# YukeWang96/GNNAdvisor_OSDI21

Measured on AMD Instinct MI355X. Metric: aggregated edges/sec, GCN sum-aggregation SpMM (SAG) hidden=64, higher is better.
Workload: dtype f32; 1 GPU; reddit-like power-law graph, random node order; num_nodes=232965, nnz=114623790, dim=64, partSize=128, num_parts=1008217, parallelism=single GPU, call=GNNA.SAG (pybind module, reference signature, fresh output), decider=auto/mi355x, column_phases=16, build_id=0.6.1+9562461010c46275

## Files before the change

gnnadvisor_osdi21_amd/csrc/gnna_agg.hip:

```cpp
#include <hip/hip_runtime.h>

#include <algorithm>
#include <cmath>
#include <cstdint>
#include <cstdio>

#include "gnna.h"
#include "gnna_device.h"
#include "gnna_internal.h"

namespace gnna {
namespace {


__global__ void __launch_bounds__(kBlock)
prologue_kernel(float *__restrict__ Y, size_t n_floats, int D, int ldy, const int32_t *__restrict__ p2n,
                const int32_t *__restrict__ pp, int64_t P, int32_t *flag, int32_t seq, int validate, int zero_fill,
                const int32_t *__restrict__ chk_ids, int64_t chk_n, const unsigned long long *__restrict__ chk_sum,
                int32_t *stale_flag, uint32_t *__restrict__ clear_words, int n_clear)
{
    if (blockIdx.x == 0 && (int)threadIdx.x < n_clear) clear_words[threadIdx.x] = 0u;
    const unsigned fill_blocks = chk_ids ? gridDim.x - 1 : gridDim.x;
    if (blockIdx.x >= fill_blocks) {
        if (threadIdx.x < kWave) {
// ... 90 lines not shown
        const bool valid = g < P;
        int64_t lo = 0, cnt = 0;
        if (valid) {
            const int64_t r = p2n[g];
            const int64_t nxt = g + 1 < P ? (int64_t)p2n[g + 1] : N;
            const int a = pp[g], b = pp[g + 1];
            if (b < a || (g + 1 < P && nxt < r)) bad = true;
            const bool continues = g > 0 && (g % G) == 0 && p2n[g - 1] == r;
            const bool self = b <= a || continues;
            lo = self ? r : r + 1;
            int64_t hi = (self && nxt < r + 1) ? r + 1 : nxt;
            lo = lo < 0 ? 0 : lo;
            hi = hi > N ? N : hi;
            cnt = hi > lo ? hi - lo : 0;
        }
        unsigned long long m = __ballot(cnt > 0);
        while (m) {
            const int l = __builtin_ctzll(m);
            m &= m - 1;
            const int64_t lo_s = ((int64_t)__builtin_amdgcn_readlane((int)(lo >> 32), l) << 32) |
                                 (uint32_t)__builtin_amdgcn_readlane((int)lo, l);
            const int64_t cnt_s = ((int64_t)__builtin_amdgcn_readlane((int)(cnt >> 32), l) << 32) |
                                  (uint32_t)__builtin_amdgcn_readlane((int)cnt, l);
            clear_rows(lo_s, cnt_s);
        }
    }
    if (validate && bad) *flag = seq;
}

__global__ void __launch_bounds__(kBlock)
post_prologue_kernel(float *__restrict__ Y, size_t n_floats, int D, int ldy, const int32_t *flag, int32_t seq,
                     const unsigned long long *gaps)
{
    const size_t tid = (size_t)blockIdx.x * blockDim.x + threadIdx.x;
    const size_t nthreads = (size_t)gridDim.x * blockDim.x;
    auto at = [&](float *base, size_t i) -> float * {
        if (ldy == D) return base + i;
        const size_t r = i / (unsigned)D;
        return base + r * (size_t)ldy + (i - r * (unsigned)D);
    };
    if (*flag == seq) {
        for (size_t i = tid; i < n_floats; i += nthreads) *at(Y, i) = 0.f;
        return;
    }
    if (!gaps) return;
    const unsigned long long n = gaps[0] < (unsigned long long)kGapEntries ? gaps[0] : (unsigned long long)kGapEntries;
    for (unsigned long long k = 0; k < n; k++) {
        float *base = Y + (size_t)gaps[2 + 2 * k] * (size_t)ldy;
        const size_t cnt = (size_t)gaps[3 + 2 * k] * (size_t)D;
        for (size_t i = tid; i < cnt; i += nthreads) *at(base, i) = 0.f;
    }
}

__global__ void __launch_bounds__(kBlock)
scale_rows_kernel(const float *__restrict__ X, int64_t ld_in, const float *__restrict__ deg, float *__restrict__ Xs,
                  int64_t rows, int D, int ld_out)
{
    const size_t tid = (size_t)blockIdx.x * blockDim.x + threadIdx.x;
    const size_t nthreads = (size_t)gridDim.x * blockDim.x;
    typedef float f32x4 __attribute__((ext_vector_type(4)));
    const bool aligned = ((reinterpret_cast<uintptr_t>(X) | reinterpret_cast<uintptr_t>(Xs)) & 15) == 0;
    if (ld_out == D && ld_in == D && (D & 3) == 0 && aligned) {
        const size_t n4 = ((size_t)rows * (size_t)D) >> 2;
        const int d4 = D >> 2;
        for (size_t i = tid; i < n4; i += nthreads) {
            const f32x4 v = __builtin_nontemporal_load(reinterpret_cast<const f32x4 *>(X) + i);
            reinterpret_cast<f32x4 *>(Xs)[i] = deg ? v * deg[i / d4] : v;
        }
    } else if ((D & 3) == 0 && (ld_out & 3) == 0 && (ld_in & 3) == 0 && aligned) {
        const size_t n4 = ((size_t)rows * (size_t)D) >> 2;
        const unsigned d4 = (unsigned)D >> 2;
        const size_t ldo4 = (size_t)ld_out >> 2, ldi4 = (size_t)ld_in >> 2;
        for (size_t i = tid; i < n4; i += nthreads) {
            const size_t r = i / d4, c4 = i - r * d4;
            const f32x4 v = __builtin_nontemporal_load(reinterpret_cast<const f32x4 *>(X) + r * ldi4 + c4);
            reinterpret_cast<f32x4 *>(Xs)[r * ldo4 + c4] = deg ? v * deg[r] : v;
        }
    } else {
        const size_t total = (size_t)rows * (size_t)D;
        for (size_t i = tid; i < total; i += nthreads) {
            const size_t r = i / (unsigned)D, cc = i - r * (unsigned)D;
            const float v = __builtin_nontemporal_load(X + r * (size_t)ld_in + cc);
            Xs[r * (size_t)ld_out + cc] = deg ? v * deg[r] : v;
        }
    }
}


static size_t gather_footprint_bytes(int64_t num_in_rows, int ldx, int dim)
{
    return (size_t)num_in_rows * (size_t)std::min(ldx, (std::max(dim, 4) * 4 + 127) / 128 * 32) * sizeof(float);
}

thread_local int t_last_phases = 1;
thread_local int t_last_launches = 1;

double avg_lines_per_row(int64_t row_bytes, int64_t stride_bytes)
{
    int64_t lines = 0;
    for (int k = 0; k < 32; k++) {
        const int64_t o = (k * stride_bytes) % 128;
        lines += (o + row_bytes + 127) / 128;
    }
    return (double)lines / 32.0;
}

int choose_row_stride(int dim)
{
    if (dim < 2 || dim > 256) return dim;
    auto cost = [&](int stride) {
        return avg_lines_per_row((int64_t)dim * 4, (int64_t)stride * 4) * ((stride & 3) ? 1.07 : 1.0);
    };
    const double plain = cost(dim);
    int best = dim;
    double best_cost = plain * 0.93;
    const int cand[3] = {(dim + 3) / 4 * 4, (dim + 15) / 16 * 16, (dim + 31) / 32 * 32};
    for (int c : cand) {
        if (c == dim || c > 2 * dim) continue;
        const double cc = cost(c) * (1.0 + 0.02 * (double)(c - dim) / (double)dim);
        if (cc < best_cost) { best = c; best_cost = cc; }
    }
    return best;
}

int pick_row_stride(const gnna_tuning &t, int dim, bool hot_rows, int64_t num_in_rows, bool whole_call)
{
    int ldx = dim;
    if (t.pad_rows == 1 || (t.pad_rows == 0 && hot_rows)) ldx = choose_row_stride(dim);
    if (t.pad_rows == 0 && hot_rows && dim > 16 && dim <= 64 && whole_call) {
        const int gapped = 2 * ((dim * 4 + 127) / 128) * 32;
        if ((size_t)num_in_rows * (size_t)gapped * sizeof(float) <= ((size_t)160 << 20)) ldx = gapped;
    }
    if (t.pad_rows > 2 && t.pad_rows >= dim) ldx = t.pad_rows;
    return ldx;
}

}
// ... 230 lines not shown
            int64_t blocks = (num_parts + kBlock - 1) / kBlock;
            blocks = std::max<int64_t>(1, std::min<int64_t>(blocks, (int64_t)ds->num_cus * 8));
            unsigned long long *gaps = ds->gap_lists + (size_t)call_block_of(ds, stream, seq) * kGapWords;
            (void)hipMemsetAsync(gaps, 0, sizeof(unsigned long long), stream);
            const int64_t big_rows = std::max<int64_t>(64, ((int64_t)1 << 20) / std::max(1, dim * 4));
            hipLaunchKernelGGL(sparse_prologue_kernel, dim3((unsigned)blocks), dim3(kBlock), 0, stream, out, num_nodes, dim, ldy,
                               part2Node, part_pointers, num_parts, sparse_G, flag, seq, validate, gaps, big_rows);
            hipLaunchKernelGGL(post_prologue_kernel, dim3((unsigned)(ds->num_cus * 8)), dim3(kBlock), 0, stream, out,
                               n_floats, dim, ldy, flag, seq, gaps);
        } else {
            size_t work = std::max(n_floats / 4, (size_t)num_parts);
            int64_t blocks = (int64_t)((work + kBlock - 1) / kBlock);
            blocks = std::max<int64_t>(1, std::min<int64_t>(blocks, (int64_t)ds->num_cus * 8));
            hipLaunchKernelGGL(prologue_kernel, dim3((unsigned)blocks + (chk_sum ? 1u : 0u)), dim3(kBlock), 0, stream, out, n_floats,
                               dim, ldy, part2Node, part_pointers, num_parts, flag, seq, validate, zero_fill,
                               chk_sum ? column_index : nullptr, chk_n, chk_sum, stale_flag, clear_words, n_clear);
        }
        hipError_t e = hipGetLastError();
        if (e != hipSuccess) return fail(GNNA_ERR_HIP, "prologue launch: %s", hipGetErrorString(e));
        profile_record(prof_call, 1, stream);
        return GNNA_OK;
    };
    if (num_parts == 0) {
        rc = run_prologue(0);
        if (rc != GNNA_OK || !relu || !accumulate_into_out) return rc;
        StreamLaunch e0;
        e0.mode = mode; e0.Y = out; e0.p2n = part2Node; e0.P = 0; e0.D = dim; e0.ldy = ldy; e0.relu = true; e0.num_out_rows = num_nodes;
        e0.flag = flag; e0.seq = seq; e0.cnt = nullptr; e0.B = 1; e0.plain_ok = false; e0.G = 1;
        return launch_stream_epilogue_only(e0, stream);
    }

    const int64_t window_rows = (num_in_rows + num_windows - 1) / num_windows;

    const int64_t est_edges = num_parts * (int64_t)(tune.avg_degree > 0 ? std::min(partSize, tune.avg_degree) : partSize / 2 + 1);
    const bool hot_rows = est_edges >= 32 * num_in_rows && (size_t)num_in_rows * (size_t)dim * sizeof(float) <= ((size_t)1 << 30);
    const bool prescale = mode == MODE_GCN && (tune.gcn_prescale == 1 || (tune.gcn_prescale == 0 && hot_rows));
    const int want = dim < 4 ? 4 : pick_row_stride(tune, dim, hot_rows, num_in_rows, !windowed);
    bool direct = !prescale && dim >= 4;
    if (direct && want != dim && ld_in != want) {
        const bool aligned16 = (reinterpret_cast<uintptr_t>(input) & 15) == 0 && (ld_in & 3) == 0;
        const int gapped = 2 * ((dim * 4 + 127) / 128) * 32;
        if (want == gapped && dim > 16 && dim <= 64)
            direct = (ld_in % gapped) == 0 && (reinterpret_cast<uintptr_t>(input) % ((size_t)gapped * 4)) == 0;
        else
            direct = aligned16 && avg_lines_per_row((int64_t)dim * 4, ld_in * 4) <= avg_lines_per_row((int64_t)dim * 4, (int64_t)want * 4) + 1e-9;
    }
    const int ldx = direct ? (int)ld_in : want;
    const float *X = input;
    const float *row_scale = nullptr;
    float eps = epsilon;
    const size_t x_bytes = (size_t)num_in_rows * (size_t)ldx * sizeof(float);
    const size_t foot_bytes = gather_footprint_bytes(num_in_rows, ldx, dim);
    const bool wide = x_bytes > 0xffffffffull;
    if (!direct) {
        void *xs = nullptr;
        rc = get_workspace(ds, stream, 1, x_bytes, &xs);
        if (rc != GNNA_OK) return rc;
        const int64_t r0 = std::min<int64_t>((int64_t)win_begin * window_rows, num_in_rows);
        const int64_t r1 = std::min<int64_t>((int64_t)win_end * window_rows, num_in_rows);
        const size_t s_bytes = (size_t)(r1 - r0) * (size_t)dim * sizeof(float);
        int64_t sblocks = (int64_t)((s_bytes / 16 + kBlock - 1) / kBlock);
        sblocks = std::max<int64_t>(1, std::min<int64_t>(sblocks, (int64_t)ds->num_cus * 8));
        hipLaunchKernelGGL(scale_rows_kernel, dim3((unsigned)sblocks), dim3(kBlock), 0, stream,
                           input + (size_t)r0 * (size_t)ld_in, ld_in, prescale ? degrees_in + r0 : nullptr,
                           static_cast<float *>(xs) + (size_t)r0 * ldx, r1 - r0, dim, ldx);
        hipError_t es = hipGetLastError();
        if (es != hipSuccess) return fail(GNNA_ERR_HIP, "staging launch: %s", hipGetErrorString(es));
        X = static_cast<const float *>(xs);
        if (prescale) {
            row_scale = degrees;
            eps = 1.f;
            mode = MODE_GIN;
        }
    }

    int B = 1;
    const uint8_t *cnt = nullptr;
    int S = kMaxSlices;
    int win_lo = 0, win_hi = 0;
    SlicePlan plan;
    const bool can_slice = num_parts >= 1024 && num_in_rows >= 64 && foot_bytes >= ((size_t)2 << 20);
    if (windowed) {
        rc = get_slice_plan(ds, stream, column_index, part_pointers, part2Node, num_parts, num_in_rows, true, false, &plan,
                            (uint32_t)std::max<int64_t>(1, window_rows));
        if (rc != GNNA_OK) return rc;
        if (!plan.cnt || !plan.stats.valid)
            return fail(GNNA_ERR_UNSUPPORTED, "the windowed aggregation needs its window counts, which cannot be built inside a "
                                              "stream capture: run the sequence once before capturing it");
        if (plan.stats.unsorted > 0)
            return fail(GNNA_ERR_UNSUPPORTED, "windowed aggregation: the column ids of %.0f neighbor-groups are not in increasing "
                                              "order (sort the ids of every row, as the loader's CSR has them)", plan.stats.unsorted);
        cnt = plan.cnt; S = plan.S; B = 1;
        win_lo = win_begin; win_hi = win_end == num_windows ? S : win_end;
    } else {
        if (tune.column_phases >= 2 && num_in_rows >= kMaxSlices) {
            B = std::min(tune.column_phases, kMaxSlices);
            rc = get_slice_plan(ds, stream, column_index, part_pointers, part2Node, num_parts, num_in_rows, false, false, &plan);
            if (rc != GNNA_OK) return rc;
        } else if (tune.column_phases == 0 && can_slice && foot_bytes >= ((size_t)6 << 20)) {
            rc = get_slice_plan(ds, stream, column_index, part_pointers, part2Node, num_parts, num_in_rows, true, false, &plan);
            if (rc != GNNA_OK) return rc;
            if (plan.cnt && plan.stats.valid)
                B = choose_slices(plan.stats, foot_bytes, plan.S, plan.slice_rows, num_nodes, num_in_rows == num_nodes,
                                  tune.nonlocal_ids == 1);
        }
        cnt = plan.cnt;
        if (cnt) S = plan.S;
        if (!cnt || B < 2) { B = 1; cnt = nullptr; }
    }

    const int auto_Bs = (cnt && !windowed && plan.stats.valid)
                            ? sweep_auto_phases(tune, mode, dim, foot_bytes, num_nodes, num_in_rows, plan.stats, B, ds->num_cus,
                                                tune.deterministic == 1, partSize) : 0;
    if (mode != MODE_EDGE && cnt && !windowed && dim >= 4 && (tune.sweep == 1 || auto_Bs > 0) && tune.deterministic != 1 &&
        sweep_supports(mode, dim, x_bytes)) {
        int Bs = B;
        if (auto_Bs > 0) {
            Bs = std::min(auto_Bs, S);
        } else if (tune.column_phases < 2) {
            Bs = std::max(2, std::min(std::min(std::min(16, 2 * B), std::max(2, partSize / 4)), S));
        }
        const int32_t *sw_ids = nullptr; const uint32_t *sw_off = nullptr;
        if (plan.handle && (tune.pack_ids == 1 || (tune.pack_ids == 0 && plan.pinned)) && tune.xcd_remap != 0) {
            rc = get_packed_ids(ds, stream, plan.handle, Bs, kWave, true, false, &sw_ids, &sw_off, &chk_sum, &chk_n, stale_flag, seq,
                                tune.ids_check_every);
            if (rc != GNNA_OK) return rc;
            if (sw_ids) count_event(CTR_PACKED_LAUNCHES);
        }
        uint32_t *sync = ds->sweep_sync + (size_t)call_block_of(ds, stream, seq) * kSweepSlotWords;
        static_assert(kXcds * 16 + 2 <= kBlock, "the prologue clears the sweep counters with one block");
        rc = run_prologue(0, sync, kXcds * 16 + 2);
        if (rc != GNNA_OK) return rc;
        SweepLaunch w;
        w.mode = mode; w.X = X; w.col = column_index; w.pp = part_pointers; w.p2n = part2Node; w.Y = out;
        w.cnt = cnt; w.row_scale = row_scale; w.flag = flag; w.seq = seq; w.trust = tune.trust_canonical ? 1 : 0; w.sync = sync;
        w.P = num_parts; w.D = dim; w.ldx = ldx; w.ldy = ldy; w.S = S; w.B = Bs;
        w.relu = relu; w.num_out_rows = num_nodes;
        w.U = std::max(tune.loads_in_flight, 8);
        w.rows_with_edges = plan.stats.valid ? (int64_t)std::min((double)num_nodes, plan.stats.groups) : num_nodes;
        if (tune.groups_per_chunk > 64) w.rounds = tune.groups_per_chunk / 64;
        w.slack = tune.sweep_slack; w.wgs_per_cu = tune.blocks_per_cu;
        w.dynamic = tune.xcd_remap != 0;
        w.plain_ok = !accumulate_into_out; w.eps = eps;
        w.ids_packed = sw_ids; w.item_off = sw_off; w.packed_stale = stale_flag;
        t_last_phases = Bs;
        t_last_launches = 1;
        rc = launch_sweep(ds, w, stream);
        if (rc != GNNA_OK) return rc;
        profile_record(prof_call, 2, stream);
        return GNNA_OK;
    }

    int G = std::min(64, tune.groups_per_chunk * B);
    if (mode == MODE_EDGE && cnt && !windowed && plan.handle && plan.pinned && (plan.stats.valid || tune.sweep == 1) &&
        tune.xcd_remap != 0) {
        const int Bs = sweep_phases_of_width(tune, dim, foot_bytes, x_bytes, num_nodes, num_in_rows, plan.stats, B, ds->num_cus,
                                             partSize, S);
        if (Bs >= 2) { B = Bs; G = kWave; }
    }
    t_last_phases = B;
    StreamLaunch a;
    a.mode = mode; a.X = X; a.col = column_index; a.pp = part_pointers; a.p2n = part2Node; a.Y = out;
    a.cnt = cnt; a.row_scale = row_scale; a.flag = flag; a.seq = seq;
    if (mode == MODE_EDGE) { a.deg_row = nullptr; a.deg_col = nullptr; a.edge_w = degrees_in; }
    else { a.deg_row = degrees; a.deg_col = degrees_in; }
    a.trust = tune.trust_canonical ? 1 : 0; a.P = num_parts;
    a.D = dim; a.ldx = ldx; a.ldy = ldy; a.G = G; a.U = tune.loads_in_flight; a.S = S; a.B = B;
    a.win_lo = win_lo; a.win_hi = win_hi; a.relu = relu; a.num_out_rows = num_nodes;
    t_last_launches = 1;
    a.wide = wide; a.plain_ok = (B == 1 && !accumulate_into_out && !windowed); a.xcd_remap = tune.xcd_remap != 0;
    a.eps = eps;
    if (tune.deterministic == 1 && !windowed) {
        const int G_eff = std::max(1, std::min(a.G, kWave));
        const size_t chunks = (size_t)((num_parts + G_eff - 1) / G_eff);
        const size_t part_bytes = ((chunks * 2 * (size_t)dim * sizeof(float)) + 255) & ~(size_t)255;
        const size_t stamp_bytes = chunks * 2 * sizeof(int32_t);
        void *ws = nullptr;
        rc = get_workspace(ds, stream, 2, part_bytes + stamp_bytes, &ws);
        if (rc != GNNA_OK) return rc;
        a.det = true;
        a.det_part = static_cast<float *>(ws);
        a.det_stamp = reinterpret_cast<int32_t *>(static_cast<char *>(ws) + part_bytes);
        hipError_t em = hipMemsetAsync(a.det_stamp, 0, stamp_bytes, stream);
        if (em != hipSuccess) return fail(GNNA_ERR_HIP, "deterministic schedule scratch: %s", hipGetErrorString(em));
        t_last_launches = B;
    }
    if (cnt && !windowed && plan.handle && (tune.pack_ids == 1 || (tune.pack_ids == 0 && plan.pinned))) {
        rc = get_packed_ids(ds, stream, plan.handle, B, std::max(1, std::min(a.G, kWave)), true, false, &a.ids_packed, &a.item_off,
                            &chk_sum, &chk_n, stale_flag, seq, tune.ids_check_every);
        a.packed_stale = stale_flag;
        if (rc != GNNA_OK) return rc;
        if (a.ids_packed) count_event(CTR_PACKED_LAUNCHES);
    }
    const bool sparse = !a.det && a.plain_ok && tune.zero_fill != 2 &&
                        (tune.zero_fill == 1 || n_floats * sizeof(float) >= ((size_t)32 << 20));
    rc = run_prologue(sparse ? std::max(1, std::min(a.G, kWave)) : 0);
    if (rc != GNNA_OK) return rc;
    rc = launch_stream(a, stream);
    if (rc != GNNA_OK) return rc;
    profile_record(prof_call, 2, stream);
    return GNNA_OK;
}

}
}
// ... 283 lines not shown
```

gnnadvisor_osdi21_amd/csrc/gnna_device.h:

```cpp
#ifndef GNNA_DEVICE_H_
#define GNNA_DEVICE_H_

#include <hip/hip_runtime.h>

#include <cstdint>
#include <type_traits>

namespace gnna {


constexpr int kWave = 64;
constexpr int kBlock = 256;
constexpr int kWavesPerBlock = kBlock / kWave;
constexpr int kXcds = 8;

enum { MODE_SAG = 0, MODE_GCN = 1, MODE_GIN = 2, MODE_SDDMM = 3, MODE_EDGE = 4 };

template <int VEC> struct VecOf;
template <> struct VecOf<1> { typedef float T; typedef float M; };
template <> struct VecOf<4> {
    typedef float T __attribute__((ext_vector_type(4)));
    typedef T M __attribute__((aligned(4)));
};

// ... 87 lines not shown
        float px, qy;
        {
            auto t = __builtin_amdgcn_permlane32_swap(__float_as_uint(acc[0]), __float_as_uint(acc[2]), false, false);
            px = __uint_as_float(t[0]) + __uint_as_float(t[1]);
            t = __builtin_amdgcn_permlane32_swap(__float_as_uint(acc[1]), __float_as_uint(acc[3]), false, false);
            qy = __uint_as_float(t[0]) + __uint_as_float(t[1]);
        }
        float val;
        {
            auto t = __builtin_amdgcn_permlane16_swap(__float_as_uint(px), __float_as_uint(qy), false, false);
            val = __uint_as_float(t[0]) + __uint_as_float(t[1]);
        }
        if constexpr (LPR <= 8) val += row_ror<8>(val);
        if constexpr (LPR <= 4) val += row_ror<4>(val);
        if constexpr (MODE == MODE_GIN) val *= scale;
        r[0] = val;
    } else {
#pragma unroll
        for (int k = 0; k < 4; k++) {
            float s = slot_reduce<LPR>(acc[k]);
            if constexpr (MODE == MODE_GIN) s *= scale;
            r[k] = s;
        }
    }
    return r;
}

__device__ __forceinline__ unsigned long long sample_checksum(const int32_t *__restrict__ ids, int64_t n, int lane)
{
    unsigned long long sum = 0;
    if (n > 0) {
        uint32_t v[16];
#pragma unroll
        for (int k = 0; k < 16; k++) {
            const int i = k * 64 + lane;
            v[k] = (uint32_t)ids[(int64_t)(((unsigned long long)i * (unsigned long long)n) >> 10)];
        }
#pragma unroll
        for (int k = 0; k < 16; k++) sum += (unsigned long long)v[k] * (unsigned long long)(2 * (k * 64 + lane) + 1);
    }
    for (int d = 32; d > 0; d >>= 1) sum += __shfl_xor(sum, d);
    return sum;
}

__device__ __forceinline__ unsigned long long graph_checksum(const int32_t *__restrict__ ids, int64_t n,
                                                             const int32_t *__restrict__ pp, int64_t P, int lane)
{
    const unsigned long long a = sample_checksum(ids, n, lane);
    const unsigned long long b = sample_checksum(pp, P + 1, lane);
    const unsigned long long last = (unsigned long long)(uint32_t)pp[P];
    return a ^ ((b + last) * 0x9E3779B97F4A7C15ull);
}

}

#endif
```

gnnadvisor_osdi21_amd/csrc/gnna_internal.h:

```cpp
#ifndef GNNA_INTERNAL_H_
#define GNNA_INTERNAL_H_

#include <hip/hip_runtime.h>

#include <atomic>
#include <cstddef>
#include <cstdint>
#include <map>
#include <utility>
#include <vector>

#include "gnna.h"

namespace gnna {

int fail(int code, const char *fmt, ...) __attribute__((format(printf, 2, 3)));

int host_thread_budget(int cap);

void apply_graph_hints(const void *column_index, int dim, gnna_tuning *tune);

struct Workspace {
    void *ptr = nullptr;
    size_t bytes = 0;
// ... 82 lines not shown
       CTR_COUNT = 10 };
void count_event(int which);

struct StreamLaunch {
    int mode;
    const float *X; const int32_t *col; const int32_t *pp; const int32_t *p2n; float *Y;
    const uint8_t *cnt;
    const float *row_scale;
    const float *deg_row; const float *deg_col;
    const float *A = nullptr;
    const float *edge_w = nullptr;
    const int32_t *flag; int32_t seq; int32_t trust;
    int64_t P;
    int D, ldx, G, U, S, B;
    int lda = 0;
    int ldy = 0;
    int win_lo = 0, win_hi = 0;
    bool relu = false;
    int64_t num_out_rows = 0;
    bool wide, plain_ok, xcd_remap;
    float eps;
    bool det = false;
    float *det_part = nullptr; int32_t *det_stamp = nullptr;
    const int32_t *ids_packed = nullptr; const uint32_t *item_off = nullptr;
    const int32_t *packed_stale = nullptr;
};
int launch_stream(const StreamLaunch &a, hipStream_t stream);
int launch_stream_epilogue_only(const StreamLaunch &a, hipStream_t stream);

struct SweepLaunch {
    int mode;
    const float *X; const int32_t *col; const int32_t *pp; const int32_t *p2n; float *Y;
    const uint8_t *cnt;
    const float *row_scale;
    const int32_t *flag; int32_t seq; int32_t trust;
    uint32_t *sync;
    int64_t P;
    int D, ldx, U, S, B;
    int ldy = 0;
    bool relu = false;
    int64_t num_out_rows = 0;
    int rounds = 0;
    int64_t rows_with_edges = 0;
    int slack = 0;
    int wgs_per_cu = 0;
    bool dynamic = true;
    bool plain_ok;
    float eps;
    const int32_t *ids_packed = nullptr; const uint32_t *item_off = nullptr;
    const int32_t *packed_stale = nullptr;
};
bool sweep_supports(int mode, int dim, size_t x_bytes);
int sweep_acc_rows(int dim, int wgs_per_cu);
int launch_sweep(DeviceState *ds, const SweepLaunch &a, hipStream_t stream);
int sweep_auto_phases(const gnna_tuning &t, int mode, int dim, size_t x_bytes, int64_t num_out_rows, int64_t num_in_rows,
                      const SlicePlanStats &st, int B, int num_cus, bool deterministic, int part_size);
constexpr int kSweepListCap = 1023;
constexpr int kSweepSlotWords = 8 * 16 + 2 + 2 * kSweepListCap;

struct X16Launch {
    int mode;
    int in_type, out_type;
    const void *input; int64_t ld_in, num_in_rows;
    const int32_t *column_index; const float *degrees_out; const float *degrees_in; float epsilon;
    const int32_t *part_pointers; const int32_t *part2Node;
    void *out; int64_t ld_out, num_out_rows;
    int dim; int64_t num_parts; int partSize;
    bool accumulate, relu, xcd_remap;
    int prof_call = -1;
};
int launch_x16(DeviceState *ds, hipStream_t stream, const X16Launch &c);
int reserve_x16(DeviceState *ds, hipStream_t stream, int64_t num_in_rows, int64_t num_out_rows, int dim);
int launch_zero_fill(DeviceState *ds, hipStream_t stream, float *out, int64_t rows, int dim, int64_t ld);

int64_t scan_tiles(int64_t n);
int launch_exclusive_scan(hipStream_t stream, int32_t *data, int64_t n, int32_t *partial);
int refuse_capture(const char *what, hipStream_t stream);

int profile_acquire_call(bool has_work);
void profile_record(int call, int which, hipStream_t stream);

}

#endif
```

gnnadvisor_osdi21_amd/csrc/gnna_sweep.hip:

```cpp
#include <hip/hip_runtime.h>

#include <algorithm>
#include <cmath>
#include <cstdint>

#include "gnna.h"
#include "gnna_device.h"
#include "gnna_internal.h"

namespace gnna {
namespace {

constexpr int kSweepIdSlots = 512;
constexpr int kSweepBlock = 1024;
constexpr int kSweepWaves = kSweepBlock / kWave;
constexpr int kSweepLockWords = 128;

template <int LPR, int WGS> constexpr int acc_floats()
{
    return WGS == 1 ? (LPR >= 16 ? 32768 : 28672) : (LPR >= 16 ? 15360 : 11264);
}

__device__ __forceinline__ void lds_add(float *p, float v)
{
    typedef __attribute__((address_space(3))) float lds_float;
    (void)__hip_atomic_fetch_add((lds_float *)p, v, __ATOMIC_RELAXED, __HIP_MEMORY_SCOPE_WORKGROUP);
}

struct SweepParams {
    const float *X;
    const int32_t *col;
    const int32_t *pp;
    const int32_t *p2n;
    float *Y;
    const uint8_t *cnt;
    const float *row_scale;
    const int32_t *flag;
    uint32_t *sync;
    int64_t P;
    int32_t seq;
    int32_t trust;
    int32_t D;
    int32_t ldx;
    int32_t ldy;
    int32_t relu;
    int32_t S;
    int32_t B;
    int32_t rounds;
    int32_t plain_ok;
    int32_t dynamic;
    int32_t slack;
    float eps;
    const int32_t *ids_packed;
    const uint32_t *item_off;
    const int32_t *packed_stale;
    int64_t num_chunks;
};

__device__ __forceinline__ int64_t lower_bound64(const int32_t *__restrict__ pp, int64_t P, int64_t target, int lane)
{
    int64_t lo = 0, hi = P;
    while (hi > lo) {
        const int64_t span = hi - lo;
        const int64_t idx = lo + (span * lane) / kWave;
        const bool below = (int64_t)pp[idx] < target;
        const int c = __popcll(__ballot(below));
        if (c == 0) { hi = lo; break; }
        const int64_t new_lo = lo + (span * (c - 1)) / kWave + 1;
        const int64_t new_hi = c < kWave ? lo + (span * c) / kWave : hi;
        lo = new_lo;
        hi = new_hi > new_lo ? new_hi : new_lo;
    }
    return lo;
}

__device__ __forceinline__ int64_t sweep_set_start(int64_t i, int64_t num_sets, int64_t nnz, const int32_t *__restrict__ pp,
                                                   int64_t P, bool canonical, bool align64, int lane)
{
    const int64_t target = i >= num_sets ? nnz : (nnz * i) / num_sets;
    int64_t g = i <= 0 ? 0 : (i >= num_sets ? P : (canonical ? lower_bound64(pp, P, target, lane) : (P * i) / num_sets));
    if (align64 && g < P) g &= ~(int64_t)(kWave - 1);
    return g;
}

__global__ void __launch_bounds__(kBlock)
sweep_relu_fixup_kernel(float *__restrict__ Y, int64_t N, int D, int ldy, const uint32_t *__restrict__ list,
                        const int32_t *flag, int32_t seq, int32_t trust, int whole)
{
    const int lane = threadIdx.x & (kWave - 1);
    const int64_t wave = ((int64_t)blockIdx.x * blockDim.x + threadIdx.x) >> 6;
    const int64_t nwaves = ((int64_t)gridDim.x * blockDim.x) >> 6;
    const bool canonical = trust || (*flag != seq);
    auto clamp_row = [&](int64_t r) {
        float *row = Y + (size_t)r * (size_t)ldy;
        for (int i = lane; i < D; i += kWave) row[i] = fmaxf(row[i], 0.f);
    };
    if (whole || !canonical || list[1] != 0u) {
        for (int64_t r = wave; r < N; r += nwaves) clamp_row(r);
        return;
    }
    const uint32_t n = list[0] < (uint32_t)kSweepListCap ? list[0] : (uint32_t)kSweepListCap;
    for (int64_t i = wave; i < (int64_t)n; i += nwaves) {
        const int64_t first = (int64_t)list[2 + 2 * i], cnt = (int64_t)list[3 + 2 * i];
        for (int64_t r = first; r < first + cnt && r < N; r++) clamp_row(r);
    }
}

template <int LPR, int MODE, int U, int WGS>
__global__ void __launch_bounds__(kSweepBlock) __attribute__((amdgpu_waves_per_eu(4 * WGS, 4 * WGS)))
sweep_kernel(const SweepParams p)
{
    typedef typename VecOf<4>::T VT;
    typedef typename VecOf<4>::M MT;
    constexpr int RPI = kWave / LPR;
    constexpr int RL = (kSweepIdSlots / RPI < kWave) ? kSweepIdSlots / RPI : kWave;
    static_assert(RL % U == 0, "a round is a whole number of batches");
    constexpr int ACC = acc_floats<LPR, WGS>();
    __shared__ float s_acc[ACC];
    __shared__ uint32_t s_off[kSweepWaves][RL * RPI];
    __shared__ int64_t s_g[2];
    __shared__ int s_ctl[8];
    __shared__ unsigned s_lock[kSweepLockWords];

    const int lane = threadIdx.x & (kWave - 1);
    const int wib = __builtin_amdgcn_readfirstlane((int)threadIdx.x >> 6);
    const int lslot = lane / LPR;
    const int c = lane % LPR;
    const int D = p.D;
    const bool canonical = p.trust || (*p.flag != p.seq);
    const bool stale_ids = p.ids_packed != nullptr && *p.packed_stale == p.seq;
    const char *xbase = reinterpret_cast<const char *>(p.X);
    const uint32_t row_bytes32 = (uint32_t)p.ldx * 4u;
    uint32_t *offs = s_off[wib];
    const int CAP = ACC / D;
    const unsigned long long upto = (2ull << lane) - 1ull;
    const unsigned long long above = ~upto;
// ... 337 lines not shown
            const float *src = s_acc + q * D;
            for (int i = lane; i < D; i += kWave) {
                const float val = src[i] * scale;
                if (!use_atomic) __builtin_nontemporal_store(p.relu ? fmaxf(val, 0.f) : val, dst + i);
                else unsafeAtomicAdd(dst + i, val);
            }
        }
        __syncthreads();
    }
}

typedef void (*SweepKernel)(const SweepParams);

template <int LPR, int MODE, int WGS>
SweepKernel pick_sweep_u(int u)
{
    constexpr int RPI = kWave / LPR;
    constexpr int RL = (kSweepIdSlots / RPI < kWave) ? kSweepIdSlots / RPI : kWave;
    if constexpr (RL % 16 == 0 && WGS == 1) {
        if (u >= 16) return sweep_kernel<LPR, MODE, 16, WGS>;
    }
    if constexpr (RL % 8 == 0 && WGS == 1) {
        if (u >= 8) return sweep_kernel<LPR, MODE, 8, WGS>;
    }
    return sweep_kernel<LPR, MODE, 4, WGS>;
}

template <int MODE, int WGS>
SweepKernel pick_sweep(int lpr, int u)
{
    switch (lpr) {
    case 4: return pick_sweep_u<4, MODE, WGS>(u);
    case 8: return pick_sweep_u<8, MODE, WGS>(u);
    case 16: return pick_sweep_u<16, MODE, WGS>(u);
    default: return pick_sweep_u<32, MODE, WGS>(u);
    }
}

}

int sweep_acc_rows(int dim, int wgs)
{
    const int pieces = (dim + 3) / 4;
    const int acc = wgs == 1 ? (pieces <= 8 ? acc_floats<8, 1>() : acc_floats<16, 1>())
                             : (pieces <= 8 ? acc_floats<8, 2>() : acc_floats<16, 2>());
    return std::max(1, acc / std::max(1, dim));
}

bool sweep_supports(int mode, int dim, size_t x_bytes)
{
    return (mode == MODE_SAG || mode == MODE_GIN) && dim >= 4 && dim <= 128 && x_bytes <= 0xffffffffull;
}

int launch_sweep(DeviceState *ds, const SweepLaunch &a, hipStream_t stream)
{
    SweepParams p;
    p.X = a.X; p.col = a.col; p.pp = a.pp; p.p2n = a.p2n; p.Y = a.Y; p.cnt = a.cnt; p.row_scale = a.row_scale;
    p.flag = a.flag; p.seq = a.seq; p.trust = a.trust; p.sync = a.sync;
    p.P = a.P; p.D = a.D; p.ldx = a.ldx; p.S = a.S; p.B = a.B; p.plain_ok = a.plain_ok ? 1 : 0; p.eps = a.eps;
    p.ldy = a.ldy > 0 ? a.ldy : a.D;
    p.relu = (a.relu && a.plain_ok) ? 1 : 0;
    p.slack = a.slack > 0 ? a.slack : 2;
    p.ids_packed = a.packed_stale ? a.ids_packed : nullptr; p.item_off = a.item_off; p.packed_stale = a.packed_stale;
    p.num_chunks = (a.P + kWave - 1) / kWave;
    p.dynamic = a.dynamic ? 1 : 0;
    int lpr = 4;
    const int pieces = (a.D + 3) / 4;
    while (lpr < 32 && lpr < pieces) lpr <<= 1;
    const int wgs = a.wgs_per_cu == 2 ? 2 : 1;
    SweepKernel k = wgs == 1 ? (a.mode == MODE_GIN ? pick_sweep<MODE_GIN, 1>(lpr, a.U) : pick_sweep<MODE_SAG, 1>(lpr, a.U))
                             : (a.mode == MODE_GIN ? pick_sweep<MODE_GIN, 2>(lpr, a.U) : pick_sweep<MODE_SAG, 2>(lpr, a.U));
    const int cus_per_xcd = std::max(1, ds->num_cus / kXcds);
    const unsigned grid = (unsigned)(cus_per_xcd * kXcds * wgs);
    const int cap = sweep_acc_rows(a.D, wgs);
    int R = a.rounds;
    if (R <= 0) {
        const double rows = (double)std::max<int64_t>(1, a.rows_with_edges);
        R = (int)std::max(1.0, std::ceil(rows / ((double)grid * 0.9 * (double)cap)));
    }
    p.rounds = std::min(R, 4096);
    hipLaunchKernelGGL(k, dim3(grid), dim3(kSweepBlock), 0, stream, p);
    hipError_t e = hipGetLastError();
    if (e != hipSuccess) return fail(GNNA_ERR_HIP, "sweep launch: %s", hipGetErrorString(e));
    count_event(CTR_SWEEP_LAUNCHES);
    if (a.relu) {
        const bool whole = !a.plain_ok;
        const int64_t blocks = std::max<int64_t>(1, std::min<int64_t>((a.num_out_rows + kWavesPerBlock - 1) / kWavesPerBlock, 256 * 8));
        hipLaunchKernelGGL(sweep_relu_fixup_kernel, dim3((unsigned)blocks), dim3(kBlock), 0, stream, a.Y, a.num_out_rows, a.D, p.ldy,
                           a.sync + kXcds * 16, a.flag, a.seq, a.trust, whole ? 1 : 0);
        e = hipGetLastError();
        if (e != hipSuccess) return fail(GNNA_ERR_HIP, "epilogue launch: %s", hipGetErrorString(e));
    }
    return GNNA_OK;
}

}
```

Baseline: 83.27 billion edges/s.

## Fuse staging, prologue and targeted output zeroing into one sweep pre-pass kernel

Adds a single pre-pass kernel that runs three jobs in one launch on separate block ranges: the row scaling/staging copy, the graph checksum, and a targeted zero-fill of output rows. The zero-fill covers gap rows with no parts and rows at sweep-set boundaries and beyond the accumulator cap, so the sweep's plain stores are correct without clearing the whole output. It replaces separate staging and prologue launches with one, cutting launch overhead and possibly full-output zero traffic. In exchange it adds a validation path where the last block zeroes all of Y in a single block if the graph is flagged bad. It also adds an extra done-counter word and moves the sweep geometry computation to the host so it can be shared.

```diff
diff --git a/gnnadvisor_osdi21_amd/csrc/gnna_agg.hip b/gnnadvisor_osdi21_amd/csrc/gnna_agg.hip
--- a/gnnadvisor_osdi21_amd/csrc/gnna_agg.hip
+++ b/gnnadvisor_osdi21_amd/csrc/gnna_agg.hip
@@ -166,12 +166,9 @@
     }
 }
 
-__global__ void __launch_bounds__(kBlock)
-scale_rows_kernel(const float *__restrict__ X, int64_t ld_in, const float *__restrict__ deg, float *__restrict__ Xs,
-                  int64_t rows, int D, int ld_out)
-{
-    const size_t tid = (size_t)blockIdx.x * blockDim.x + threadIdx.x;
-    const size_t nthreads = (size_t)gridDim.x * blockDim.x;
+__device__ __forceinline__ void scale_rows(const float *__restrict__ X, int64_t ld_in, const float *__restrict__ deg,
+                                           float *__restrict__ Xs, int64_t rows, int D, int ld_out, size_t tid, size_t nthreads)
+{
     typedef float f32x4 __attribute__((ext_vector_type(4)));
     const bool aligned = ((reinterpret_cast<uintptr_t>(X) | reinterpret_cast<uintptr_t>(Xs)) & 15) == 0;
     if (ld_out == D && ld_in == D && (D & 3) == 0 && aligned) {
@@ -197,6 +194,131 @@
             const float v = __builtin_nontemporal_load(X + r * (size_t)ld_in + cc);
             Xs[r * (size_t)ld_out + cc] = deg ? v * deg[r] : v;
         }
+    }
+}
+
+__global__ void __launch_bounds__(kBlock)
+scale_rows_kernel(const float *__restrict__ X, int64_t ld_in, const float *__restrict__ deg, float *__restrict__ Xs,
+                  int64_t rows, int D, int ld_out)
+{
+    scale_rows(X, ld_in, deg, Xs, rows, D, ld_out, (size_t)blockIdx.x * blockDim.x + threadIdx.x, (size_t)gridDim.x * blockDim.x);
+}
+
+struct PrepassParams {
+    const float *X; const float *deg; float *Xs;
+    int64_t ld_in, stage_rows; int ld_out;
+    float *Y; int64_t N; int D, ldy;
+    const int32_t *p2n, *pp; int64_t P;
+    int32_t *flag; int32_t seq; int validate;
+    const int32_t *chk_ids; int64_t chk_n; const unsigned long long *chk_sum; int32_t *stale_flag;
+    uint32_t *clear_words; int n_clear; uint32_t *done;
+    unsigned walk_blocks, stage_blocks;
+    int64_t num_sets, big_rows; int cap, align64;
+};
+
+__global__ void __launch_bounds__(kBlock)
+sweep_prepass_kernel(const PrepassParams p)
+{
+    typedef float f32x4 __attribute__((ext_vector_type(4)));
+    const int lane = threadIdx.x & (kWave - 1);
+    const int D = p.D, ldy = p.ldy;
+    float *__restrict__ Y = p.Y;
+    const int64_t N = p.N, P = p.P;
+    if (blockIdx.x >= p.walk_blocks + p.stage_blocks) {
+        if (threadIdx.x < kWave) {
+            const unsigned long long then = p.chk_sum[0], distrusted = p.chk_sum[4];
+            const unsigned long long now = graph_checksum(p.chk_ids, p.chk_n, p.pp, P, (int)threadIdx.x);
+            if (threadIdx.x == 0 && (now != then || distrusted != 0ull)) *p.stale_flag = p.seq;
+        }
+    } else if (blockIdx.x >= p.walk_blocks) {
+        scale_rows(p.X, p.ld_in, p.deg, p.Xs, p.stage_rows, D, p.ld_out,
+                   (size_t)(blockIdx.x - p.walk_blocks) * blockDim.x + threadIdx.x, (size_t)p.stage_blocks * blockDim.x);
+    } else {
+        if (blockIdx.x == 0 && (int)threadIdx.x < p.n_clear) p.clear_words[threadIdx.x] = 0u;
+        const int64_t wave = ((int64_t)blockIdx.x * blockDim.x + threadIdx.x) >> 6;
+        const int64_t nwaves = ((int64_t)p.walk_blocks * blockDim.x) >> 6;
+        const bool vec_ok = ldy == D && (D & 3) == 0 && (reinterpret_cast<uintptr_t>(Y) & 15) == 0;
+        auto clear_rows = [&](int64_t lo, int64_t hi) {
+            lo = lo < 0 ? 0 : lo;
+            hi = hi > N ? N : hi;
+            if (hi <= lo) return;
+            if (vec_ok) {
+                f32x4 *b4 = reinterpret_cast<f32x4 *>(Y + (size_t)lo * (size_t)D);
+                const size_t n4 = ((size_t)(hi - lo) * (size_t)D) >> 2;
+                const f32x4 z = (f32x4)(0.f);
+                for (size_t i = lane; i < n4; i += kWave) b4[i] = z;
+            } else {
+                for (int64_t r = lo; r < hi; r++) {
+                    float *row = Y + (size_t)r * (size_t)ldy;
+                    for (int i = lane; i < D; i += kWave) row[i] = 0.f;
+                }
+            }
+        };
+        auto clear_gap = [&](int64_t lo, int64_t hi) {
+            if (hi - lo >= p.big_rows) {
+                const int64_t edge = (lo + p.big_rows - 1) / p.big_rows * p.big_rows;
+                hi = edge < hi ? edge : hi;
+            }
+            clear_rows(lo, hi);
+        };
+        if (wave == 0) clear_gap(0, (int64_t)p.p2n[0]);
+        bool bad = false;
+        for (int64_t g0 = wave * kWave; g0 < P; g0 += nwaves * kWave) {
+            const int64_t g = g0 + lane;
+            int64_t lo = 0, hi = 0;
+            if (g < P) {
+                const int64_t r = p.p2n[g];
+                const int64_t nxt = g + 1 < P ? (int64_t)p.p2n[g + 1] : N;
+                if (p.pp[g + 1] < p.pp[g] || (g + 1 < P && nxt < r)) bad = true;
+                lo = r + 1; hi = nxt;
+            }
+            unsigned long long m = __ballot(hi > lo);
+            while (m) {
+                const int l = __builtin_ctzll(m);
+                m &= m - 1;
+                const int64_t lo_s = ((int64_t)__builtin_amdgcn_readlane((int)(lo >> 32), l) << 32) |
+                                     (uint32_t)__builtin_amdgcn_readlane((int)lo, l);
+                const int64_t hi_s = ((int64_t)__builtin_amdgcn_readlane((int)(hi >> 32), l) << 32) |
+                                     (uint32_t)__builtin_amdgcn_readlane((int)hi, l);
+                clear_gap(lo_s, hi_s);
+            }
+        }
+        if (p.validate && bad) (void)__hip_atomic_exchange(p.flag, p.seq, __ATOMIC_RELAXED, __HIP_MEMORY_SCOPE_AGENT);
+        const int64_t tiles = (N + p.big_rows - 1) / p.big_rows;
+        for (int64_t t = wave; t < tiles; t += nwaves) {
+            const int64_t b = t * p.big_rows;
+            const int64_t g = lower_bound64(p.p2n, P, b, lane);
+            const int64_t prev = g > 0 ? (int64_t)p.p2n[g - 1] : -1;
+            const int64_t next = g < P ? (int64_t)p.p2n[g] : N;
+            if (prev < b && next > b && next - (prev + 1) >= p.big_rows) clear_rows(b, b + p.big_rows < next ? b + p.big_rows : next);
+        }
+        const int64_t nnz = (int64_t)p.pp[P];
+        for (int64_t s = wave; s < p.num_sets; s += nwaves) {
+            const int64_t g_lo = sweep_set_start(s, p.num_sets, nnz, p.pp, P, true, p.align64 != 0, lane);
+            const int64_t g_hi = sweep_set_start(s + 1, p.num_sets, nnz, p.pp, P, true, p.align64 != 0, lane);
+            if (g_hi <= g_lo || g_lo < 0 || g_hi > P) continue;
+            const int64_t row_first = p.p2n[g_lo], row_last = p.p2n[g_hi - 1];
+            if (g_lo > 0 && (int64_t)p.p2n[g_lo - 1] == row_first) clear_rows(row_first, row_first + 1);
+            if (g_hi < P && (int64_t)p.p2n[g_hi] == row_last) clear_rows(row_last, row_last + 1);
+            clear_rows(row_first + p.cap, row_last + 1);
+        }
+    }
+    if (!p.validate) return;
+    __shared__ int s_last;
+    __syncthreads();
+    if (threadIdx.x == 0) {
+        __threadfence();
+        const uint32_t ticket = __hip_atomic_fetch_add(p.done, 1u, __ATOMIC_ACQ_REL, __HIP_MEMORY_SCOPE_AGENT);
+        s_last = ticket == gridDim.x - 1u ? 1 : 0;
+    }
+    __syncthreads();
+    if (!s_last) return;
+    if (threadIdx.x == 0) __hip_atomic_store(p.done, 0u, __ATOMIC_RELAXED, __HIP_MEMORY_SCOPE_AGENT);
+    if (__hip_atomic_load(p.flag, __ATOMIC_ACQUIRE, __HIP_MEMORY_SCOPE_AGENT) != p.seq) return;
+    const size_t n_floats = (size_t)N * (size_t)D;
+    for (size_t i = threadIdx.x; i < n_floats; i += kBlock) {
+        const size_t r = i / (unsigned)D;
+        Y[r * (size_t)ldy + (i - r * (unsigned)D)] = 0.f;
     }
 }
 
@@ -533,20 +655,16 @@
     const size_t x_bytes = (size_t)num_in_rows * (size_t)ldx * sizeof(float);
     const size_t foot_bytes = gather_footprint_bytes(num_in_rows, ldx, dim);
     const bool wide = x_bytes > 0xffffffffull;
+    const int64_t stage_r0 = std::min<int64_t>((int64_t)win_begin * window_rows, num_in_rows);
+    const int64_t stage_r1 = std::min<int64_t>((int64_t)win_end * window_rows, num_in_rows);
+    int64_t sblocks = 0;
     if (!direct) {
         void *xs = nullptr;
         rc = get_workspace(ds, stream, 1, x_bytes, &xs);
         if (rc != GNNA_OK) return rc;
-        const int64_t r0 = std::min<int64_t>((int64_t)win_begin * window_rows, num_in_rows);
-        const int64_t r1 = std::min<int64_t>((int64_t)win_end * window_rows, num_in_rows);
-        const size_t s_bytes = (size_t)(r1 - r0) * (size_t)dim * sizeof(float);
-        int64_t sblocks = (int64_t)((s_bytes / 16 + kBlock - 1) / kBlock);
+        const size_t s_bytes = (size_t)(stage_r1 - stage_r0) * (size_t)dim * sizeof(float);
+        sblocks = (int64_t)((s_bytes / 16 + kBlock - 1) / kBlock);
         sblocks = std::max<int64_t>(1, std::min<int64_t>(sblocks, (int64_t)ds->num_cus * 8));
-        hipLaunchKernelGGL(scale_rows_kernel, dim3((unsigned)sblocks), dim3(kBlock), 0, stream,
-                           input + (size_t)r0 * (size_t)ld_in, ld_in, prescale ? degrees_in + r0 : nullptr,
-                           static_cast<float *>(xs) + (size_t)r0 * ldx, r1 - r0, dim, ldx);
-        hipError_t es = hipGetLastError();
-        if (es != hipSuccess) return fail(GNNA_ERR_HIP, "staging launch: %s", hipGetErrorString(es));
         X = static_cast<const float *>(xs);
         if (prescale) {
             row_scale = degrees;
@@ -554,6 +672,17 @@
             mode = MODE_GIN;
         }
     }
+    const float *stage_src = input + (size_t)stage_r0 * (size_t)ld_in;
+    const float *stage_deg = prescale ? degrees_in + stage_r0 : nullptr;
+    float *stage_dst = direct ? nullptr : const_cast<float *>(X) + (size_t)stage_r0 * ldx;
+    auto stage_rows = [&]() -> int {
+        if (direct) return GNNA_OK;
+        hipLaunchKernelGGL(scale_rows_kernel, dim3((unsigned)sblocks), dim3(kBlock), 0, stream, stage_src, ld_in, stage_deg,
+                           stage_dst, stage_r1 - stage_r0, dim, ldx);
+        hipError_t es = hipGetLastError();
+        if (es != hipSuccess) return fail(GNNA_ERR_HIP, "staging launch: %s", hipGetErrorString(es));
+        return GNNA_OK;
+    };
 
     int B = 1;
     const uint8_t *cnt = nullptr;
@@ -609,9 +738,7 @@
             if (sw_ids) count_event(CTR_PACKED_LAUNCHES);
         }
         uint32_t *sync = ds->sweep_sync + (size_t)call_block_of(ds, stream, seq) * kSweepSlotWords;
-        static_assert(kXcds * 16 + 2 <= kBlock, "the prologue clears the sweep counters with one block");
-        rc = run_prologue(0, sync, kXcds * 16 + 2);
-        if (rc != GNNA_OK) return rc;
+        static_assert(kXcds * 16 + 2 <= kBlock, "the pre-pass clears the sweep counters with one block");
         SweepLaunch w;
         w.mode = mode; w.X = X; w.col = column_index; w.pp = part_pointers; w.p2n = part2Node; w.Y = out;
         w.cnt = cnt; w.row_scale = row_scale; w.flag = flag; w.seq = seq; w.trust = tune.trust_canonical ? 1 : 0; w.sync = sync;
@@ -624,14 +751,41 @@
         w.dynamic = tune.xcd_remap != 0;
         w.plain_ok = !accumulate_into_out; w.eps = eps;
         w.ids_packed = sw_ids; w.item_off = sw_off; w.packed_stale = stale_flag;
+        const SweepGeometry geo = sweep_geometry(ds, w);
+        if (w.plain_ok && tune.zero_fill != 2) {
+            PrepassParams q;
+            q.X = stage_src; q.deg = stage_deg; q.Xs = stage_dst; q.ld_in = ld_in; q.stage_rows = stage_r1 - stage_r0; q.ld_out = ldx;
+            q.Y = out; q.N = num_nodes; q.D = dim; q.ldy = ldy; q.p2n = part2Node; q.pp = part_pointers; q.P = num_parts;
+            q.flag = flag; q.seq = seq; q.validate = tune.trust_canonical ? 0 : 1;
+            q.chk_ids = chk_sum ? column_index : nullptr; q.chk_n = chk_n; q.chk_sum = chk_sum; q.stale_flag = stale_flag;
+            q.clear_words = sync; q.n_clear = kXcds * 16 + 2; q.done = sync + kSweepDoneWord;
+            q.num_sets = (int64_t)geo.grid * geo.rounds; q.cap = geo.cap; q.align64 = geo.align64 ? 1 : 0;
+            q.big_rows = std::max<int64_t>(64, ((int64_t)1 << 20) / std::max(1, dim * 4));
+            const int64_t walk_waves = std::max(std::max((num_parts + kWave - 1) / kWave, q.num_sets),
+                                                (num_nodes + q.big_rows - 1) / q.big_rows);
+            q.walk_blocks = (unsigned)std::max<int64_t>(1, std::min<int64_t>((walk_waves + kWavesPerBlock - 1) / kWavesPerBlock,
+                                                                              (int64_t)ds->num_cus * 4));
+            q.stage_blocks = (unsigned)sblocks;
+            hipLaunchKernelGGL(sweep_prepass_kernel, dim3(q.walk_blocks + q.stage_blocks + (chk_sum ? 1u : 0u)), dim3(kBlock), 0, stream, q);
+            hipError_t e = hipGetLastError();
+            if (e != hipSuccess) return fail(GNNA_ERR_HIP, "pre-pass launch: %s", hipGetErrorString(e));
+            profile_record(prof_call, 1, stream);
+        } else {
+            rc = stage_rows();
+            if (rc != GNNA_OK) return rc;
+            rc = run_prologue(0, sync, kXcds * 16 + 2);
+            if (rc != GNNA_OK) return rc;
+        }
         t_last_phases = Bs;
         t_last_launches = 1;
-        rc = launch_sweep(ds, w, stream);
+        rc = launch_sweep(ds, w, geo, stream);
         if (rc != GNNA_OK) return rc;
         profile_record(prof_call, 2, stream);
         return GNNA_OK;
     }
 
+    rc = stage_rows();
+    if (rc != GNNA_OK) return rc;
     int G = std::min(64, tune.groups_per_chunk * B);
     if (mode == MODE_EDGE && cnt && !windowed && plan.handle && plan.pinned && (plan.stats.valid || tune.sweep == 1) &&
         tune.xcd_remap != 0) {
diff --git a/gnnadvisor_osdi21_amd/csrc/gnna_device.h b/gnnadvisor_osdi21_amd/csrc/gnna_device.h
--- a/gnnadvisor_osdi21_amd/csrc/gnna_device.h
+++ b/gnnadvisor_osdi21_amd/csrc/gnna_device.h
@@ -163,6 +163,33 @@
     return a ^ ((b + last) * 0x9E3779B97F4A7C15ull);
 }
 
+
+__device__ __forceinline__ int64_t lower_bound64(const int32_t *__restrict__ pp, int64_t P, int64_t target, int lane)
+{
+    int64_t lo = 0, hi = P;
+    while (hi > lo) {
+        const int64_t span = hi - lo;
+        const int64_t idx = lo + (span * lane) / kWave;
+        const bool below = (int64_t)pp[idx] < target;
+        const int c = __popcll(__ballot(below));
+        if (c == 0) { hi = lo; break; }
+        const int64_t new_lo = lo + (span * (c - 1)) / kWave + 1;
+        const int64_t new_hi = c < kWave ? lo + (span * c) / kWave : hi;
+        lo = new_lo;
+        hi = new_hi > new_lo ? new_hi : new_lo;
+    }
+    return lo;
+}
+
+__device__ __forceinline__ int64_t sweep_set_start(int64_t i, int64_t num_sets, int64_t nnz, const int32_t *__restrict__ pp,
+                                                   int64_t P, bool canonical, bool align64, int lane)
+{
+    const int64_t target = i >= num_sets ? nnz : (nnz * i) / num_sets;
+    int64_t g = i <= 0 ? 0 : (i >= num_sets ? P : (canonical ? lower_bound64(pp, P, target, lane) : (P * i) / num_sets));
+    if (align64 && g < P) g &= ~(int64_t)(kWave - 1);
+    return g;
+}
+
 }
 
 #endif
diff --git a/gnnadvisor_osdi21_amd/csrc/gnna_internal.h b/gnnadvisor_osdi21_amd/csrc/gnna_internal.h
--- a/gnnadvisor_osdi21_amd/csrc/gnna_internal.h
+++ b/gnnadvisor_osdi21_amd/csrc/gnna_internal.h
@@ -158,11 +158,14 @@
 };
 bool sweep_supports(int mode, int dim, size_t x_bytes);
 int sweep_acc_rows(int dim, int wgs_per_cu);
-int launch_sweep(DeviceState *ds, const SweepLaunch &a, hipStream_t stream);
+struct SweepGeometry { unsigned grid; int rounds; int wgs; int cap; bool align64; };
+SweepGeometry sweep_geometry(const DeviceState *ds, const SweepLaunch &a);
+int launch_sweep(DeviceState *ds, const SweepLaunch &a, const SweepGeometry &geo, hipStream_t stream);
 int sweep_auto_phases(const gnna_tuning &t, int mode, int dim, size_t x_bytes, int64_t num_out_rows, int64_t num_in_rows,
                       const SlicePlanStats &st, int B, int num_cus, bool deterministic, int part_size);
 constexpr int kSweepListCap = 1023;
-constexpr int kSweepSlotWords = 8 * 16 + 2 + 2 * kSweepListCap;
+constexpr int kSweepDoneWord = 8 * 16 + 2 + 2 * kSweepListCap;
+constexpr int kSweepSlotWords = kSweepDoneWord + 2;
 
 struct X16Launch {
     int mode;
diff --git a/gnnadvisor_osdi21_amd/csrc/gnna_sweep.hip b/gnnadvisor_osdi21_amd/csrc/gnna_sweep.hip
--- a/gnnadvisor_osdi21_amd/csrc/gnna_sweep.hip
+++ b/gnnadvisor_osdi21_amd/csrc/gnna_sweep.hip
@@ -57,31 +57,6 @@
     int64_t num_chunks;
 };
 
-__device__ __forceinline__ int64_t lower_bound64(const int32_t *__restrict__ pp, int64_t P, int64_t target, int lane)
-{
-    int64_t lo = 0, hi = P;
-    while (hi > lo) {
-        const int64_t span = hi - lo;
-        const int64_t idx = lo + (span * lane) / kWave;
-        const bool below = (int64_t)pp[idx] < target;
-        const int c = __popcll(__ballot(below));
-        if (c == 0) { hi = lo; break; }
-        const int64_t new_lo = lo + (span * (c - 1)) / kWave + 1;
-        const int64_t new_hi = c < kWave ? lo + (span * c) / kWave : hi;
-        lo = new_lo;
-        hi = new_hi > new_lo ? new_hi : new_lo;
-    }
-    return lo;
-}
-
-__device__ __forceinline__ int64_t sweep_set_start(int64_t i, int64_t num_sets, int64_t nnz, const int32_t *__restrict__ pp,
-                                                   int64_t P, bool canonical, bool align64, int lane)
-{
-    const int64_t target = i >= num_sets ? nnz : (nnz * i) / num_sets;
-    int64_t g = i <= 0 ? 0 : (i >= num_sets ? P : (canonical ? lower_bound64(pp, P, target, lane) : (P * i) / num_sets));
-    if (align64 && g < P) g &= ~(int64_t)(kWave - 1);
-    return g;
-}
 
 __global__ void __launch_bounds__(kBlock)
 sweep_relu_fixup_kernel(float *__restrict__ Y, int64_t N, int D, int ldy, const uint32_t *__restrict__ list,
@@ -525,8 +500,26 @@
     return (mode == MODE_SAG || mode == MODE_GIN) && dim >= 4 && dim <= 128 && x_bytes <= 0xffffffffull;
 }
 
-int launch_sweep(DeviceState *ds, const SweepLaunch &a, hipStream_t stream)
-{
+SweepGeometry sweep_geometry(const DeviceState *ds, const SweepLaunch &a)
+{
+    SweepGeometry g;
+    g.wgs = a.wgs_per_cu == 2 ? 2 : 1;
+    const int cus_per_xcd = std::max(1, ds->num_cus / kXcds);
+    g.grid = (unsigned)(cus_per_xcd * kXcds * g.wgs);
+    g.cap = sweep_acc_rows(a.D, g.wgs);
+    int R = a.rounds;
+    if (R <= 0) {
+        const double rows = (double)std::max<int64_t>(1, a.rows_with_edges);
+        R = (int)std::max(1.0, std::ceil(rows / ((double)g.grid * 0.9 * (double)g.cap)));
+    }
+    g.rounds = std::min(R, 4096);
+    g.align64 = a.packed_stale != nullptr && a.ids_packed != nullptr;
+    return g;
+}
+
+int launch_sweep(DeviceState *ds, const SweepLaunch &a, const SweepGeometry &geo, hipStream_t stream)
+{
+    (void)ds;
     SweepParams p;
     p.X = a.X; p.col = a.col; p.pp = a.pp; p.p2n = a.p2n; p.Y = a.Y; p.cnt = a.cnt; p.row_scale = a.row_scale;
     p.flag = a.flag; p.seq = a.seq; p.trust = a.trust; p.sync = a.sync;
@@ -534,24 +527,17 @@
     p.ldy = a.ldy > 0 ? a.ldy : a.D;
     p.relu = (a.relu && a.plain_ok) ? 1 : 0;
     p.slack = a.slack > 0 ? a.slack : 2;
-    p.ids_packed = a.packed_stale ? a.ids_packed : nullptr; p.item_off = a.item_off; p.packed_stale = a.packed_stale;
+    p.ids_packed = geo.align64 ? a.ids_packed : nullptr; p.item_off = a.item_off; p.packed_stale = a.packed_stale;
     p.num_chunks = (a.P + kWave - 1) / kWave;
     p.dynamic = a.dynamic ? 1 : 0;
     int lpr = 4;
     const int pieces = (a.D + 3) / 4;
     while (lpr < 32 && lpr < pieces) lpr <<= 1;
-    const int wgs = a.wgs_per_cu == 2 ? 2 : 1;
+    const int wgs = geo.wgs;
     SweepKernel k = wgs == 1 ? (a.mode == MODE_GIN ? pick_sweep<MODE_GIN, 1>(lpr, a.U) : pick_sweep<MODE_SAG, 1>(lpr, a.U))
                              : (a.mode == MODE_GIN ? pick_sweep<MODE_GIN, 2>(lpr, a.U) : pick_sweep<MODE_SAG, 2>(lpr, a.U));
-    const int cus_per_xcd = std::max(1, ds->num_cus / kXcds);
-    const unsigned grid = (unsigned)(cus_per_xcd * kXcds * wgs);
-    const int cap = sweep_acc_rows(a.D, wgs);
-    int R = a.rounds;
-    if (R <= 0) {
-        const double rows = (double)std::max<int64_t>(1, a.rows_with_edges);
-        R = (int)std::max(1.0, std::ceil(rows / ((double)grid * 0.9 * (double)cap)));
-    }
-    p.rounds = std::min(R, 4096);
+    const unsigned grid = geo.grid;
+    p.rounds = geo.rounds;
     hipLaunchKernelGGL(k, dim3(grid), dim3(kSweepBlock), 0, stream, p);
     hipError_t e = hipGetLastError();
     if (e != hipSuccess) return fail(GNNA_ERR_HIP, "sweep launch: %s", hipGetErrorString(e));
```

Measured after the change: 73.22 billion edges/s. 0.879x the previous value.
